# csyxwei/FFWM

Measured on AMD Instinct MI355X. Metric: train img/s (128x128, full FFWM GAN step), higher is better.
Workload: dtype f32; 1 GPU; BASELINE configs[2]: full FFWM train step (netG+netD+flowNetF+flowNetB, all losses, 3x Adam), synthetic MultiPIE-shaped 128x128; batch_per_gpu=8, global_batch=8, parallelism=dp1, grad_buckets=10, bucket_MiB=64

## Files before the change

### ffwm_amd/csrc/conv_bwd.hip

```cpp
#include "common.hpp"

namespace ffwm {
namespace {

typedef float f32x16 __attribute__((ext_vector_type(16)));

struct WgGeo {
    int C, H, W;
    int K, Ho, Wo;
    int stride, pad;
    int N;
    int P;
    int chunks_per_img;
    int chunks;
    int total_chunks;
    unsigned a_bytes, x_bytes;
};

constexpr int kPC = 32;
constexpr int kWAP = kPC + 1;
constexpr int kWBP = 65;

template <int R, int S>
__global__ void __launch_bounds__(kBlock)
conv_wgrad_generic_kernel(const float* __restrict__ a, const float* __restrict__ x, float* __restrict__ dw, const WgGeo g) {
    constexpr int RS = R * S;
    __shared__ float As[64 * kWAP];
    __shared__ float Bs[kPC * kWBP];
    const int lane = threadIdx.x & 63, wave = threadIdx.x >> 6;
    const int l31 = lane & 31, half = lane >> 5;
    const int wm = wave >> 1, wn = wave & 1;
    const int n0 = blockIdx.x * 64, k0 = blockIdx.y * 64;
    constexpr unsigned kOobOff = 0xFFFFFFF0u;
    const rsrc_t ra_ = make_rsrc(a, g.a_bytes);
    const rsrc_t rx_ = make_rsrc(x, g.x_bytes);
    const int HW = g.H * g.W;

    const int kk = threadIdx.x & 31, j0 = threadIdx.x >> 5;
    unsigned arow[8];
    int bc[8], br[8], bs[8];
#pragma unroll
    for (int i = 0; i < 8; ++i) {
        const int j = j0 + 8 * i;
        arow[i] = (k0 + j < g.K) ? static_cast<unsigned>(k0 + j) * static_cast<unsigned>(g.P) : kOobOff;
        const int n = n0 + j;
        if (n < g.N) {
            const int c = n / RS, rs = n - c * RS;
            bc[i] = c; br[i] = rs / S - g.pad; bs[i] = rs % S - g.pad;
        } else {
            bc[i] = -1; br[i] = 0; bs[i] = 0;
        }
    }

    const int ch_begin = blockIdx.z * g.chunks;
    const int ch_end = min(g.total_chunks, ch_begin + g.chunks);

    auto fetch = [&](int ch, float (&va)[8], float (&vb)[8]) {
        const int b = ch / g.chunks_per_img;
        const int p = (ch - b * g.chunks_per_img) * kPC + kk;
        const bool pin = p < g.P;
        const int oy = p / g.Wo, ox = p - oy * g.Wo;
        const int iy0 = oy * g.stride, ix0 = ox * g.stride;
        const unsigned abase = static_cast<unsigned>(b) * static_cast<unsigned>(g.K) * static_cast<unsigned>(g.P) + p;
        const unsigned xbase = static_cast<unsigned>(b) * static_cast<unsigned>(g.C) * static_cast<unsigned>(HW);
#pragma unroll
        for (int i = 0; i < 8; ++i) va[i] = buf_ld<float>(ra_, (pin && arow[i] != kOobOff) ? (abase + arow[i]) * 4u : kOobOff);
#pragma unroll
        for (int i = 0; i < 8; ++i) {
            const int iy = iy0 + br[i], ix = ix0 + bs[i];
            const bool ok = pin && bc[i] >= 0 && iy >= 0 && iy < g.H && ix >= 0 && ix < g.W;
            vb[i] = buf_ld<float>(rx_, ok ? (xbase + static_cast<unsigned>(bc[i]) * static_cast<unsigned>(HW) + static_cast<unsigned>(iy * g.W + ix)) * 4u
                                          : kOobOff);
        }
    };
    auto commit = [&](const float (&va)[8], const float (&vb)[8]) {
#pragma unroll
        for (int i = 0; i < 8; ++i) As[(j0 + 8 * i) * kWAP + kk] = va[i];
#pragma unroll
        for (int i = 0; i < 8; ++i) Bs[kk * kWBP + j0 + 8 * i] = vb[i];
    };

    f32x16 acc;
#pragma unroll
    for (int r = 0; r < 16; ++r) acc[r] = 0.f;
    auto compute = [&]() {
        const float* ap = As + (wm * 32 + l31) * kWAP + half;
        const float* bp = Bs + half * kWBP + wn * 32 + l31;
#pragma unroll
        for (int q = 0; q < kPC / 2; ++q)
            acc = __builtin_amdgcn_mfma_f32_32x32x2f32(ap[2 * q], bp[2 * q * kWBP], acc, 0, 0, 0);
    };

    float a0[8], b0[8], a1[8], b1[8];
    if (ch_begin < ch_end) fetch(ch_begin, a0, b0);
    if (ch_begin + 1 < ch_end) fetch(ch_begin + 1, a1, b1);
    for (int ch = ch_begin; ch < ch_end; ch += 2) {
        __syncthreads();
        commit(a0, b0);
        __syncthreads();
        if (ch + 2 < ch_end) fetch(ch + 2, a0, b0);
        compute();
        if (ch + 1 >= ch_end) break;
        __syncthreads();
        commit(a1, b1);
        __syncthreads();
        if (ch + 3 < ch_end) fetch(ch + 3, a1, b1);
        compute();
    }

    const int n = n0 + wn * 32 + l31;
    if (n >= g.N) return;
#pragma unroll
    for (int r = 0; r < 16; ++r) {
        const int k = k0 + wm * 32 + (r & 3) + 8 * (r >> 2) + 4 * half;
        if (k < g.K) atomic_add(dw + static_cast<size_t>(k) * g.N + n, acc[r]);
    }
}


struct Wg2Geo {
    int C, H, W, K, Ho, Wo, stride, pad;
    int N, P, HW;
    int total_px;
    int chunks_total;
    int chunks;
    int nz;
    unsigned a_bytes, x_bytes;
    FastDiv divP, divWo;
};

constexpr int kW2PC = 32;
constexpr int kW2P = 36;

template <int R, int S, int WM, int WN>
__global__ void __launch_bounds__(kBlock, 2)
conv_wgrad_tile_kernel(const float* __restrict__ a, const float* __restrict__ x, float* __restrict__ dw, float* __restrict__ gbias,
                       const Wg2Geo g) {
    constexpr int RS = R * S;
    constexpr int TM = 64 * WM, TN = 64 * WN;
    constexpr int NQA = TM * 8 / kBlock;
    constexpr int NXB = TN / 8;
    typedef float f32x4 __attribute__((ext_vector_type(4)));
    extern __shared__ __attribute__((aligned(16))) unsigned char smem_raw[];
    float* lds = reinterpret_cast<float*>(smem_raw);
    const int lane = threadIdx.x & 63, wave = threadIdx.x >> 6;
    const int l31 = lane & 31, half = lane >> 5;
    const int wm = wave >> 1, wn = wave & 1;
    const int n0 = blockIdx.x * TN, k0 = blockIdx.y * TM;
    constexpr unsigned kOobOff = 0xFFFFFFF0u;
    const rsrc_t ra_ = make_rsrc(a, g.a_bytes);
    const rsrc_t rx_ = make_rsrc(x, g.x_bytes);

    const int q8 = threadIdx.x & 7, arow0 = threadIdx.x >> 3;
    unsigned arow_off[NQA];
#pragma unroll
    for (int i = 0; i < NQA; ++i) {
        const int k = k0 + arow0 + 32 * i;
        arow_off[i] = k < g.K ? static_cast<unsigned>(k) * static_cast<unsigned>(g.P) : kOobOff;
    }
    const int kk = threadIdx.x & 31, xcol0 = threadIdx.x >> 5;
    int coloff[NXB];
    unsigned colsh[NXB];
#pragma unroll
    for (int i = 0; i < NXB; ++i) {
        const int n = n0 + xcol0 + 8 * i;
        const bool cin = n < g.N;
        const int nc = cin ? n : 0;
        const int c = nc / RS, rs = nc - c * RS;
        const int r = rs / S, sx = rs - r * S;
        coloff[i] = c * g.HW + r * g.W + sx;
        colsh[i] = cin ? static_cast<unsigned>(8 * r + sx) : 31u;
    }

    const int ch_begin = blockIdx.z * g.chunks;
    const int ch_end = min(g.chunks_total, ch_begin + g.chunks);
    const bool want_bias = gbias != nullptr && blockIdx.x == 0;

    f32x4 va[NQA];
    float vx[NXB];
    float bsum[NQA];
#pragma unroll
    for (int i = 0; i < NQA; ++i) bsum[i] = 0.f;

    unsigned a_base, a_pin;
    int x_base;
    int x_inv;
    auto prep = [&](int ch) {
        {
            const unsigned gq = static_cast<unsigned>(ch) * kW2PC + q8 * 4;
            const unsigned b = fast_div(gq, g.divP);
            const unsigned p = gq - b * static_cast<unsigned>(g.P);
            a_pin = 0u - static_cast<unsigned>(gq < static_cast<unsigned>(g.total_px));
            a_base = b * static_cast<unsigned>(g.K) * static_cast<unsigned>(g.P) + p;
        }
        {
            const unsigned gq = static_cast<unsigned>(ch) * kW2PC + kk;
            const unsigned b = fast_div(gq, g.divP);
            const unsigned p = gq - b * static_cast<unsigned>(g.P);
            const unsigned pin = static_cast<unsigned>(gq < static_cast<unsigned>(g.total_px));
            const int oy = static_cast<int>(fast_div(p, g.divWo)), ox = static_cast<int>(p) - oy * g.Wo;
            const int iy0 = oy * g.stride - g.pad, ix0 = ox * g.stride - g.pad;
            unsigned rmask = 0, smask = 0;
#pragma unroll
            for (int r = 0; r < R; ++r) rmask |= static_cast<unsigned>(static_cast<unsigned>(iy0 + r) < static_cast<unsigned>(g.H)) << r;
#pragma unroll
            for (int q = 0; q < S; ++q) smask |= static_cast<unsigned>(static_cast<unsigned>(ix0 + q) < static_cast<unsigned>(g.W)) << q;
            unsigned taps = 0;
#pragma unroll
            for (int r = 0; r < R; ++r) taps |= (smask & (0u - ((rmask >> r) & 1u))) << (8 * r);
            x_inv = static_cast<int>(~(taps & (0u - pin)));
            x_base = static_cast<int>(b) * g.C * g.HW + iy0 * g.W + ix0;
        }
    };
    auto issue_a = [&](int i) {
        const unsigned live = a_pin & (0u - static_cast<unsigned>(arow_off[i] != kOobOff));
        const unsigned off = (((a_base + arow_off[i]) * 4u) & live) | (kOobOff & ~live);
        const u32x4 v = __builtin_amdgcn_raw_buffer_load_b128(ra_, off, 0, 0);
        va[i][0] = __uint_as_float(v.x); va[i][1] = __uint_as_float(v.y); va[i][2] = __uint_as_float(v.z); va[i][3] = __uint_as_float(v.w);
    };
    auto issue_x = [&](int i) {
        const unsigned dead = static_cast<unsigned>(__builtin_amdgcn_sbfe(x_inv, colsh[i], 1u));
        vx[i] = buf_ld<float>(rx_, (static_cast<unsigned>(x_base + coloff[i]) << 2) | dead);
    };
    auto fetch = [&](int ch) {
        prep(ch);
#pragma unroll
        for (int i = 0; i < NQA; ++i) issue_a(i);
#pragma unroll
        for (int i = 0; i < NXB; ++i) issue_x(i);
    };
    auto commit = [&](int buf) {
        float* As = lds + buf * (TM + TN) * kW2P;
        float* Xs = As + TM * kW2P;
#pragma unroll
        for (int i = 0; i < NQA; ++i) {
            *reinterpret_cast<f32x4*>(As + (arow0 + 32 * i) * kW2P + q8 * 4) = va[i];
            if (want_bias) bsum[i] += (va[i][0] + va[i][1]) + (va[i][2] + va[i][3]);
        }
#pragma unroll
        for (int i = 0; i < NXB; ++i) Xs[(xcol0 + 8 * i) * kW2P + kk] = vx[i];
    };

    f32x16 acc[WM][WN];
#pragma unroll
    for (int i = 0; i < WM; ++i)
#pragma unroll
        for (int j = 0; j < WN; ++j)
#pragma unroll
            for (int r = 0; r < 16; ++r) acc[i][j][r] = 0.f;

    auto compute = [&](int buf, int next) {
        const float* As = lds + buf * (TM + TN) * kW2P;
        const float* Xs = As + TM * kW2P;
        const float* ap = As + (wm * 32 * WM + l31) * kW2P + 4 * half;
        const float* bp = Xs + (wn * 32 * WN + l31) * kW2P + 4 * half;
        if (next >= 0) prep(next);
#pragma unroll
        for (int gq = 0; gq < kW2PC / 8; ++gq) {
            f32x4 av[WM], bv[WN];
#pragma unroll
            for (int i = 0; i < WM; ++i) av[i] = *reinterpret_cast<const f32x4*>(ap + i * 32 * kW2P + 8 * gq);
#pragma unroll
            for (int j = 0; j < WN; ++j) bv[j] = *reinterpret_cast<const f32x4*>(bp + j * 32 * kW2P + 8 * gq);
            if (next >= 0) {
#pragma unroll
                for (int i = 0; i < NQA; ++i)
                    if (i % 4 == gq) issue_a(i);
#pragma unroll
                for (int i = 0; i < NXB; ++i)
                    if (i / (NXB / 4) == gq) issue_x(i);
            }
#pragma unroll
            for (int q = 0; q < 4; ++q)
#pragma unroll
                for (int i = 0; i < WM; ++i)
#pragma unroll
                    for (int j = 0; j < WN; ++j)
                        acc[i][j] = __builtin_amdgcn_mfma_f32_32x32x2f32(av[i][q], bv[j][q], acc[i][j], 0, 0, 0);
            __builtin_amdgcn_sched_barrier(0);
        }
    };

    if (ch_begin < ch_end) {
        fetch(ch_begin);
        commit(0);
        if (ch_begin + 1 < ch_end) fetch(ch_begin + 1);
        __syncthreads();
        for (int ch = ch_begin; ch < ch_end; ++ch) {
            const int cur = (ch - ch_begin) & 1;
            if (ch + 1 < ch_end) commit(cur ^ 1);
            compute(cur, ch + 2 < ch_end ? ch + 2 : -1);
            __syncthreads();
        }
    }

#pragma unroll
    for (int j = 0; j < WN; ++j) {
        const int n = n0 + wn * 32 * WN + j * 32 + l31;
        if (n >= g.N) continue;
#pragma unroll
        for (int i = 0; i < WM; ++i)
#pragma unroll
            for (int r = 0; r < 16; ++r) {
                const int k = k0 + wm * 32 * WM + i * 32 + (r & 3) + 8 * (r >> 2) + 4 * half;
                if (k >= g.K) continue;
                float* d = dw + static_cast<size_t>(k) * g.N + n;
                if (g.nz > 1) atomic_add(d, acc[i][j][r]);
                else *d = acc[i][j][r];
            }
    }
    if (want_bias) {
#pragma unroll
        for (int i = 0; i < NQA; ++i) {
            float v = bsum[i];
            v += __shfl_xor(v, 1, 64);
            v += __shfl_xor(v, 2, 64);
            v += __shfl_xor(v, 4, 64);
            const int k = k0 + arow0 + 32 * i;
            if (q8 == 0 && k < g.K) {
                if (g.nz > 1) atomic_add(gbias + k, v);
                else gbias[k] = v;
            }
        }
    }
}

}
}

using namespace ffwm;

extern "C" int ffwm_conv2d_wgrad(const void* rows, const void* gathered, void* grad_weight, int64_t B, int64_t K, int64_t Ho,
                                 int64_t Wo, int64_t C, int64_t H, int64_t W, int kernel, int stride, int pad, int dtype, void* stream) {
    const char* fn = "ffwm_conv2d_wgrad";
    FFWM_REQUIRE(dtype == FFWM_F32, FFWM_ERR_DTYPE, "%s: float32 only", fn);
    FFWM_REQUIRE(rows && gathered && grad_weight, FFWM_ERR_ARG, "%s: NULL tensor pointer", fn);
    FFWM_REQUIRE(B > 0 && K > 0 && C > 0 && Ho > 0 && Wo > 0 && H > 0 && W > 0, FFWM_ERR_ARG, "%s: sizes must be positive", fn);
    FFWM_REQUIRE((kernel == 1 || kernel == 3 || kernel == 4) && (stride == 1 || stride == 2) && pad >= 0 && pad < kernel, FFWM_ERR_ARG,
                 "%s: 1x1 / 3x3 / 4x4 kernels with stride 1 / 2 only", fn);
    FFWM_REQUIRE(Ho == (H + 2 * pad - kernel) / stride + 1 && Wo == (W + 2 * pad - kernel) / stride + 1, FFWM_ERR_ARG,
                 "%s: the row tensor's plane (%lld x %lld) is not the output plane of this convolution over %lld x %lld", fn,
                 (long long)Ho, (long long)Wo, (long long)H, (long long)W);
    FFWM_REQUIRE(B * K * Ho * Wo < (1LL << 29) && B * C * H * W < (1LL << 29), FFWM_ERR_SIZE, "%s: tensors must stay below 2 GiB", fn);
    WgGeo g;
    g.C = static_cast<int>(C); g.H = static_cast<int>(H); g.W = static_cast<int>(W);
    g.K = static_cast<int>(K); g.Ho = static_cast<int>(Ho); g.Wo = static_cast<int>(Wo);
    g.stride = stride; g.pad = pad;
    g.N = g.C * kernel * kernel;
    g.P = g.Ho * g.Wo;
    g.chunks_per_img = (g.P + kPC - 1) / kPC;
    g.total_chunks = static_cast<int>(B) * g.chunks_per_img;
    g.a_bytes = static_cast<unsigned>(B * K * Ho * Wo * 4);
    g.x_bytes = static_cast<unsigned>(B * C * H * W * 4);
    const int n_tiles = (g.N + 63) / 64, k_tiles = (g.K + 63) / 64;
    int64_t slices = (1024 + static_cast<int64_t>(n_tiles) * k_tiles - 1) / (static_cast<int64_t>(n_tiles) * k_tiles);
    if (slices > g.total_chunks / 4) slices = g.total_chunks / 4;
    if (slices < 1) slices = 1;
    g.chunks = static_cast<int>((g.total_chunks + slices - 1) / slices);
    const unsigned nz = static_cast<unsigned>((g.total_chunks + g.chunks - 1) / g.chunks);
    hipStream_t st = static_cast<hipStream_t>(stream);
    const double flops = 2.0 * B * g.P * static_cast<double>(g.K) * g.N;
    const double bytes = 4.0 * (static_cast<double>(B) * K * g.P + static_cast<double>(B) * C * H * W + static_cast<double>(K) * g.N);
    LaunchScope ls("conv_wgrad_mfma_generic", st, bytes, flops);
    const dim3 grid(static_cast<unsigned>(n_tiles), static_cast<unsigned>(k_tiles), nz);
    const float* a = static_cast<const float*>(rows);
    const float* x = static_cast<const float*>(gathered);
    float* dw = static_cast<float*>(grad_weight);
    if (kernel == 3) hipLaunchKernelGGL((conv_wgrad_generic_kernel<3, 3>), grid, dim3(kBlock), 0, st, a, x, dw, g);
    else if (kernel == 4) hipLaunchKernelGGL((conv_wgrad_generic_kernel<4, 4>), grid, dim3(kBlock), 0, st, a, x, dw, g);
    else hipLaunchKernelGGL((conv_wgrad_generic_kernel<1, 1>), grid, dim3(kBlock), 0, st, a, x, dw, g);
    return check_launch(fn);
}

extern "C" int ffwm_conv2d_wgrad_tiled(const void* rows, const void* gathered, void* grad_weight, void* grad_bias, int64_t B, int64_t K,
                                       int64_t Ho, int64_t Wo, int64_t C, int64_t H, int64_t W, int kernel, int stride, int pad,
                                       int prezeroed, int dtype, void* stream) {
    const char* fn = "ffwm_conv2d_wgrad_tiled";
    FFWM_REQUIRE(dtype == FFWM_F32, FFWM_ERR_DTYPE, "%s: float32 only", fn);
    FFWM_REQUIRE(rows && gathered && grad_weight, FFWM_ERR_ARG, "%s: NULL tensor pointer", fn);
    FFWM_REQUIRE(B > 0 && K > 0 && C > 0 && Ho > 0 && Wo > 0 && H > 0 && W > 0, FFWM_ERR_ARG, "%s: sizes must be positive", fn);
    FFWM_REQUIRE((kernel == 1 || kernel == 3 || kernel == 4) && (stride == 1 || stride == 2) && pad >= 0 && pad < kernel, FFWM_ERR_ARG,
                 "%s: 1x1 / 3x3 / 4x4 kernels with stride 1 / 2 only", fn);
    FFWM_REQUIRE(Ho == (H + 2 * pad - kernel) / stride + 1 && Wo == (W + 2 * pad - kernel) / stride + 1, FFWM_ERR_ARG,
                 "%s: the row tensor's plane (%lld x %lld) is not the output plane of this convolution over %lld x %lld", fn,
                 (long long)Ho, (long long)Wo, (long long)H, (long long)W);
    FFWM_REQUIRE((Ho * Wo) % 4 == 0, FFWM_ERR_ARG, "%s: the row tensor's plane must hold a multiple of 4 pixels", fn);
    FFWM_REQUIRE((reinterpret_cast<uintptr_t>(rows) & 15) == 0, FFWM_ERR_ARG, "%s: the row tensor must be 16-byte aligned", fn);
    FFWM_REQUIRE(B * K * Ho * Wo < (1LL << 29) && B * C * H * W < (1LL << 29), FFWM_ERR_SIZE, "%s: tensors must stay below 2 GiB", fn);
    Wg2Geo g;
    g.C = static_cast<int>(C); g.H = static_cast<int>(H); g.W = static_cast<int>(W);
    g.K = static_cast<int>(K); g.Ho = static_cast<int>(Ho); g.Wo = static_cast<int>(Wo);
    g.stride = stride; g.pad = pad;
    g.N = g.C * kernel * kernel;
    g.P = g.Ho * g.Wo;
    g.HW = g.H * g.W;
    g.total_px = static_cast<int>(B) * g.P;
    g.chunks_total = (g.total_px + kW2PC - 1) / kW2PC;
    g.a_bytes = static_cast<unsigned>(B * K * Ho * Wo * 4);
    g.x_bytes = static_cast<unsigned>(B * C * H * W * 4);
    g.divP = make_fast_div(static_cast<unsigned>(g.P));
    g.divWo = make_fast_div(static_cast<unsigned>(g.Wo));
    const int64_t wg_target = options().conv_wgrad_slice_target > 0 ? options().conv_wgrad_slice_target : 512;
    int wmt = 1, wnt = 1;
    double best = 1e30;
    for (int cm = 1; cm <= 2; ++cm)
        for (int cn = 1; cn <= 2; ++cn) {
            if ((cm == 2 && g.K <= 64) || (cn == 2 && g.N <= 64)) continue;
            const int64_t t = static_cast<int64_t>((g.K + 64 * cm - 1) / (64 * cm)) * ((g.N + 64 * cn - 1) / (64 * cn));
            int64_t sl = t >= wg_target ? 1 : wg_target / t;
            if (sl > g.chunks_total / 4) sl = g.chunks_total / 4;
            if (sl < 1) sl = 1;
            const int64_t per = (g.chunks_total + sl - 1) / sl;
            const int64_t nzc = (g.chunks_total + per - 1) / per;
            const int64_t rounds = (t * nzc + 511) / 512;
            const double est = rounds * (per * cm * cn * (cm * cn == 1 ? 1.6 : (cm * cn == 2 ? 1.25 : 1.0)) + 6.0 + (nzc > 1 ? 2.0 * cm * cn : 0.0));
            if (est < best) { best = est; wmt = cm; wnt = cn; }
        }
    const int k_tiles = (g.K + 64 * wmt - 1) / (64 * wmt), n_tiles = (g.N + 64 * wnt - 1) / (64 * wnt);
    const int64_t tiles = static_cast<int64_t>(k_tiles) * n_tiles;
    int64_t slices = tiles >= wg_target ? 1 : wg_target / tiles;
    if (slices > g.chunks_total / 4) slices = g.chunks_total / 4;
    if (slices < 1 || options().conv_wgrad_unsliced) slices = 1;
    g.chunks = static_cast<int>((g.chunks_total + slices - 1) / slices);
    g.nz = (g.chunks_total + g.chunks - 1) / g.chunks;
    hipStream_t st = static_cast<hipStream_t>(stream);
    float* dw = static_cast<float*>(grad_weight);
    float* gb = static_cast<float*>(grad_bias);
    if (g.nz > 1 && !prezeroed) {
        const size_t nw = static_cast<size_t>(g.K) * g.N;
        const bool joined = gb == dw + nw;
        if (zero_fill(dw, sizeof(float) * (nw + (joined ? static_cast<size_t>(g.K) : 0)), st)) return FFWM_ERR_LAUNCH;
        if (gb && !joined && zero_fill(gb, sizeof(float) * static_cast<size_t>(g.K), st)) return FFWM_ERR_LAUNCH;
    }
    const double flops = 2.0 * B * g.P * static_cast<double>(g.K) * g.N;
    const double bytes = 4.0 * (static_cast<double>(B) * K * g.P + static_cast<double>(B) * C * H * W + static_cast<double>(K) * g.N);
    LaunchScope ls("conv_wgrad_mfma_tiled", st, bytes, flops);
    const dim3 grid(static_cast<unsigned>(n_tiles), static_cast<unsigned>(k_tiles), static_cast<unsigned>(g.nz));
    const float* a = static_cast<const float*>(rows);
    const float* x = static_cast<const float*>(gathered);
#define FFWM_WG2(RR, MM, NN)                                                                                                  \
    do {                                                                                                                      \
        auto kfn = conv_wgrad_tile_kernel<RR, RR, MM, NN>;                                                                    \
        const size_t lds = 2u * (64 * MM + 64 * NN) * kW2P * sizeof(float);                                                   \
        allow_large_lds(reinterpret_cast<const void*>(kfn));                                                                  \
        hipLaunchKernelGGL(kfn, grid, dim3(kBlock), lds, st, a, x, dw, gb, g);                                                \
    } while (0)
#define FFWM_WG2_K(RR)                                                                                                        \
    do {                                                                                                                      \
        if (wmt == 2 && wnt == 2) FFWM_WG2(RR, 2, 2);                                                                         \
        else if (wmt == 2) FFWM_WG2(RR, 2, 1);                                                                                \
        else if (wnt == 2) FFWM_WG2(RR, 1, 2);                                                                                \
        else FFWM_WG2(RR, 1, 1);                                                                                              \
    } while (0)
    if (kernel == 3) FFWM_WG2_K(3);
    else if (kernel == 4) FFWM_WG2_K(4);
    else FFWM_WG2_K(1);
#undef FFWM_WG2_K
#undef FFWM_WG2
    return check_launch(fn);
}
```

Before: 214.3 img/s.

## Add row-staged 3x3 wgrad kernel that reuses input halo rows in LDS

Adds a new weight-gradient kernel for 3x3 pad-1 convolutions. It stages whole input row windows, with halo columns, per channel into LDS and derives all nine taps from that shared copy, so the input no longer has to be gathered once per (c,r,s) column. The N tiling changes from 64 im2col columns to 7 channels (63 columns), and the tile-size search and the dispatch are updated to match. In exchange it adds extra index math, LDS padding, a wasted column per tile and a larger code path, with possible register pressure given launch bounds of 2.

```diff
diff --git a/ffwm_amd/csrc/conv_bwd.hip b/ffwm_amd/csrc/conv_bwd.hip
--- a/ffwm_amd/csrc/conv_bwd.hip
+++ b/ffwm_amd/csrc/conv_bwd.hip
@@ -298,6 +298,270 @@
     for (int j = 0; j < WN; ++j) {
         const int n = n0 + wn * 32 * WN + j * 32 + l31;
         if (n >= g.N) continue;
+#pragma unroll
+        for (int i = 0; i < WM; ++i)
+#pragma unroll
+            for (int r = 0; r < 16; ++r) {
+                const int k = k0 + wm * 32 * WM + i * 32 + (r & 3) + 8 * (r >> 2) + 4 * half;
+                if (k >= g.K) continue;
+                float* d = dw + static_cast<size_t>(k) * g.N + n;
+                if (g.nz > 1) atomic_add(d, acc[i][j][r]);
+                else *d = acc[i][j][r];
+            }
+    }
+    if (want_bias) {
+#pragma unroll
+        for (int i = 0; i < NQA; ++i) {
+            float v = bsum[i];
+            v += __shfl_xor(v, 1, 64);
+            v += __shfl_xor(v, 2, 64);
+            v += __shfl_xor(v, 4, 64);
+            const int k = k0 + arow0 + 32 * i;
+            if (q8 == 0 && k < g.K) {
+                if (g.nz > 1) atomic_add(gbias + k, v);
+                else gbias[k] = v;
+            }
+        }
+    }
+}
+
+struct WgRowsGeo {
+    Wg2Geo g;
+    int cols, lcols;
+    int wr;
+    int qr;
+    int rp, cp;
+};
+
+constexpr int kWgRowsMaxLds = 80 * 1024;
+
+template <int STRIDE, int WN> struct WgRowsCfg {
+    static constexpr int NCH = 7 * WN;
+    static constexpr int NQX = STRIDE == 1 ? WN : WN + 1;
+    static constexpr int NHX = (STRIDE == 1 && WN == 2) ? 2 : 1;
+    static constexpr int NS = STRIDE == 1 ? 2 : 1;
+};
+
+template <int STRIDE, int WM, int WN>
+__global__ void __launch_bounds__(kBlock, 2)
+conv_wgrad_rows_kernel(const float* __restrict__ a, const float* __restrict__ x, float* __restrict__ dw, float* __restrict__ gbias,
+                       const WgRowsGeo gr) {
+    typedef WgRowsCfg<STRIDE, WN> Cfg;
+    constexpr int TM = 64 * WM;
+    constexpr int NCH = Cfg::NCH, NQX = Cfg::NQX, NHX = Cfg::NHX, NS = Cfg::NS;
+    constexpr int NQA = TM * 8 / kBlock;
+    typedef float f32x4 __attribute__((ext_vector_type(4)));
+    const Wg2Geo& g = gr.g;
+    extern __shared__ __attribute__((aligned(16))) unsigned char smem_raw[];
+    float* lds = reinterpret_cast<float*>(smem_raw);
+    float* const xs0 = lds + 2 * TM * kW2P;
+    const int xbuf = (NCH * gr.cp + 31) & ~31;
+    const int zoff = 2 * xbuf;
+    const int lane = threadIdx.x & 63, wave = threadIdx.x >> 6;
+    const int l31 = lane & 31, half = lane >> 5;
+    const int wm = wave >> 1, wn = wave & 1;
+    const int c0 = blockIdx.x * NCH, k0 = blockIdx.y * TM;
+    constexpr unsigned kOobOff = 0xFFFFFFF0u;
+    constexpr int kNoRow = 0x40000000;
+    const rsrc_t ra_ = make_rsrc(a, g.a_bytes);
+    const rsrc_t rx_ = make_rsrc(x, g.x_bytes);
+
+    const int q8 = threadIdx.x & 7, arow0 = threadIdx.x >> 3;
+    unsigned arow_off[NQA];
+#pragma unroll
+    for (int i = 0; i < NQA; ++i) {
+        const int k = k0 + arow0 + 32 * i;
+        arow_off[i] = k < g.K ? static_cast<unsigned>(k) * static_cast<unsigned>(g.P) : kOobOff;
+    }
+    int xq_g[NQX], xq_row[NQX], xq_l[NQX];
+    {
+        const int per_c = gr.wr * gr.qr, ntask = NCH * per_c;
+#pragma unroll
+        for (int i = 0; i < NQX; ++i) {
+            const int t = threadIdx.x + kBlock * i;
+            const bool in = t < ntask;
+            const int tt = in ? t : 0;
+            const int c = tt / per_c, rem = tt - c * per_c;
+            const int row = rem / gr.qr, q = rem - row * gr.qr;
+            xq_g[i] = c * g.HW + row * g.W + 4 * q;
+            xq_row[i] = (in && c0 + c < g.C) ? row : kNoRow;
+            xq_l[i] = in ? c * gr.cp + row * gr.rp + 1 + 4 * q : zoff;
+        }
+    }
+    int xh_g[NHX], xh_row[NHX], xh_l[NHX];
+    unsigned xh_right = 0;
+    {
+        const int per_c = gr.wr * NS, ntask = NCH * per_c;
+        const int xr = gr.cols * STRIDE;
+#pragma unroll
+        for (int i = 0; i < NHX; ++i) {
+            const int t = threadIdx.x + kBlock * i;
+            const bool in = t < ntask;
+            const int tt = in ? t : 0;
+            const int c = tt / per_c, rem = tt - c * per_c;
+            const int row = rem / NS, side = rem - row * NS;
+            xh_g[i] = c * g.HW + row * g.W + (side ? xr : -1);
+            xh_row[i] = (in && c0 + c < g.C) ? row : kNoRow;
+            xh_l[i] = in ? c * gr.cp + row * gr.rp + (side ? xr + 1 : 0) : zoff;
+            xh_right |= static_cast<unsigned>(side) << i;
+        }
+    }
+    int lb[2][WN];
+#pragma unroll
+    for (int j = 0; j < WN; ++j) {
+        const int n = wn * 32 * WN + j * 32 + l31;
+        const int c = n / 9, rs = n - 9 * c;
+        const int r = rs / 3, s = rs - 3 * r;
+        const int o = r * gr.rp + s;
+        lb[0][j] = c < NCH ? c * gr.cp + o : zoff + ((9 * NCH) & 31) + o;
+        lb[1][j] = c < NCH ? xbuf + c * gr.cp + o : zoff + ((9 * NCH) & 31) + o;
+    }
+    int poff[kW2PC / 8];
+#pragma unroll
+    for (int gq = 0; gq < kW2PC / 8; ++gq) {
+        const int px = 8 * gq + 4 * half;
+        poff[gq] = (px >> gr.lcols) * STRIDE * gr.rp + (px & (gr.cols - 1)) * STRIDE;
+    }
+
+    const int ch_begin = blockIdx.z * g.chunks;
+    const int ch_end = min(g.chunks_total, ch_begin + g.chunks);
+    const bool want_bias = gbias != nullptr && blockIdx.x == 0;
+
+    f32x4 va[NQA];
+    u32x4 vq[NQX];
+    float vh[NHX];
+    float bsum[NQA];
+#pragma unroll
+    for (int i = 0; i < NQA; ++i) bsum[i] = 0.f;
+
+    unsigned a_base, a_pin;
+    int x_base, x_iy0;
+    unsigned x_ldead, x_rdead;
+    auto prep = [&](int ch) {
+        {
+            const unsigned gq = static_cast<unsigned>(ch) * kW2PC + q8 * 4;
+            const unsigned b = fast_div(gq, g.divP);
+            const unsigned p = gq - b * static_cast<unsigned>(g.P);
+            a_pin = 0u - static_cast<unsigned>(gq < static_cast<unsigned>(g.total_px));
+            a_base = b * static_cast<unsigned>(g.K) * static_cast<unsigned>(g.P) + p;
+        }
+        {
+            const unsigned gq = static_cast<unsigned>(ch) * kW2PC;
+            const unsigned b = fast_div(gq, g.divP);
+            const unsigned p = gq - b * static_cast<unsigned>(g.P);
+            const int oy = static_cast<int>(fast_div(p, g.divWo)), ox = static_cast<int>(p) - oy * g.Wo;
+            x_iy0 = oy * STRIDE - 1;
+            x_base = (static_cast<int>(b) * g.C + c0) * g.HW + x_iy0 * g.W + ox * STRIDE;
+            x_ldead = 0u - static_cast<unsigned>(ox == 0);
+            x_rdead = 0u - static_cast<unsigned>((ox + gr.cols) * STRIDE >= g.W);
+        }
+    };
+    auto issue_a = [&](int i) {
+        const unsigned live = a_pin & (0u - static_cast<unsigned>(arow_off[i] != kOobOff));
+        const unsigned off = (((a_base + arow_off[i]) * 4u) & live) | (kOobOff & ~live);
+        const u32x4 v = __builtin_amdgcn_raw_buffer_load_b128(ra_, off, 0, 0);
+        va[i][0] = __uint_as_float(v.x); va[i][1] = __uint_as_float(v.y); va[i][2] = __uint_as_float(v.z); va[i][3] = __uint_as_float(v.w);
+    };
+    auto issue_q = [&](int i) {
+        const unsigned dead = static_cast<unsigned>(x_iy0 + xq_row[i]) < static_cast<unsigned>(g.H) ? 0u : kOobOff;
+        vq[i] = __builtin_amdgcn_raw_buffer_load_b128(rx_, (static_cast<unsigned>(x_base + xq_g[i]) << 2) | dead, 0, 0);
+    };
+    auto issue_h = [&](int i) {
+        const unsigned side = ((xh_right >> i) & 1u) ? x_rdead : x_ldead;
+        const unsigned dead = static_cast<unsigned>(x_iy0 + xh_row[i]) < static_cast<unsigned>(g.H) ? side : ~0u;
+        vh[i] = buf_ld<float>(rx_, (static_cast<unsigned>(x_base + xh_g[i]) << 2) | dead);
+    };
+    auto fetch = [&](int ch) {
+        prep(ch);
+#pragma unroll
+        for (int i = 0; i < NQA; ++i) issue_a(i);
+#pragma unroll
+        for (int i = 0; i < NQX; ++i) issue_q(i);
+#pragma unroll
+        for (int i = 0; i < NHX; ++i) issue_h(i);
+    };
+    auto commit = [&](int buf) {
+        float* As = lds + buf * TM * kW2P;
+        float* Xs = xs0 + buf * xbuf;
+#pragma unroll
+        for (int i = 0; i < NQA; ++i) {
+            *reinterpret_cast<f32x4*>(As + (arow0 + 32 * i) * kW2P + q8 * 4) = va[i];
+            if (want_bias) bsum[i] += (va[i][0] + va[i][1]) + (va[i][2] + va[i][3]);
+        }
+#pragma unroll
+        for (int i = 0; i < NQX; ++i) {
+            float* d = (xq_l[i] == zoff ? xs0 : Xs) + xq_l[i];
+            d[0] = __uint_as_float(vq[i].x); d[1] = __uint_as_float(vq[i].y); d[2] = __uint_as_float(vq[i].z); d[3] = __uint_as_float(vq[i].w);
+        }
+#pragma unroll
+        for (int i = 0; i < NHX; ++i) (xh_l[i] == zoff ? xs0 : Xs)[xh_l[i]] = vh[i];
+    };
+
+    f32x16 acc[WM][WN];
+#pragma unroll
+    for (int i = 0; i < WM; ++i)
+#pragma unroll
+        for (int j = 0; j < WN; ++j)
+#pragma unroll
+            for (int r = 0; r < 16; ++r) acc[i][j][r] = 0.f;
+
+    auto compute = [&](int buf, int next) {
+        const float* ap = lds + buf * TM * kW2P + (wm * 32 * WM + l31) * kW2P + 4 * half;
+        if (next >= 0) prep(next);
+#pragma unroll
+        for (int gq = 0; gq < kW2PC / 8; ++gq) {
+            f32x4 av[WM];
+            float bv[WN][4];
+#pragma unroll
+            for (int i = 0; i < WM; ++i) av[i] = *reinterpret_cast<const f32x4*>(ap + i * 32 * kW2P + 8 * gq);
+#pragma unroll
+            for (int j = 0; j < WN; ++j) {
+                const float* bp = xs0 + (buf ? lb[1][j] : lb[0][j]) + poff[gq];
+#pragma unroll
+                for (int q = 0; q < 4; ++q) bv[j][q] = bp[q * STRIDE];
+            }
+            if (next >= 0) {
+#pragma unroll
+                for (int i = 0; i < NQA; ++i)
+                    if (i % 4 == gq) issue_a(i);
+#pragma unroll
+                for (int i = 0; i < NQX; ++i)
+                    if (i == gq) issue_q(i);
+#pragma unroll
+                for (int i = 0; i < NHX; ++i)
+                    if (3 - i == gq) issue_h(i);
+            }
+#pragma unroll
+            for (int q = 0; q < 4; ++q)
+#pragma unroll
+                for (int i = 0; i < WM; ++i)
+#pragma unroll
+                    for (int j = 0; j < WN; ++j)
+                        acc[i][j] = __builtin_amdgcn_mfma_f32_32x32x2f32(av[i][q], bv[j][q], acc[i][j], 0, 0, 0);
+            __builtin_amdgcn_sched_barrier(0);
+        }
+    };
+
+    for (int i = threadIdx.x; i < gr.cp + 32; i += kBlock) xs0[zoff + i] = 0.f;
+    if (ch_begin < ch_end) {
+        fetch(ch_begin);
+        commit(0);
+        if (ch_begin + 1 < ch_end) fetch(ch_begin + 1);
+        __syncthreads();
+        for (int ch = ch_begin; ch < ch_end; ++ch) {
+            const int cur = (ch - ch_begin) & 1;
+            if (ch + 1 < ch_end) commit(cur ^ 1);
+            compute(cur, ch + 2 < ch_end ? ch + 2 : -1);
+            __syncthreads();
+        }
+    }
+
+#pragma unroll
+    for (int j = 0; j < WN; ++j) {
+        const int nl = wn * 32 * WN + j * 32 + l31;
+        const int c = nl / 9;
+        if (c >= NCH || c0 + c >= g.C) continue;
+        const int n = c0 * 9 + nl;
 #pragma unroll
         for (int i = 0; i < WM; ++i)
 #pragma unroll
@@ -400,13 +664,36 @@
     g.x_bytes = static_cast<unsigned>(B * C * H * W * 4);
     g.divP = make_fast_div(static_cast<unsigned>(g.P));
     g.divWo = make_fast_div(static_cast<unsigned>(g.Wo));
+    WgRowsGeo gr;
+    bool staged = false;
+    if (kernel == 3 && pad == 1 && W == Wo * stride && (reinterpret_cast<uintptr_t>(gathered) & 15) == 0) {
+        const int cols = Wo % 32 == 0 ? 32 : ((Wo >= 4 && 32 % Wo == 0 && Ho % (32 / Wo) == 0) ? static_cast<int>(Wo) : 0);
+        if (cols) {
+            gr.cols = cols;
+            gr.lcols = cols == 32 ? 5 : (cols == 16 ? 4 : (cols == 8 ? 3 : 2));
+            gr.wr = (32 / cols - 1) * stride + 3;
+            gr.qr = cols * stride / 4;
+            gr.rp = cols * stride + 2 <= 35 ? 35 : 67;
+            gr.cp = gr.wr * gr.rp;
+            gr.cp += (9 - gr.cp % 32 + 32) % 32;
+            staged = true;
+        }
+    }
+    auto rows_lds = [&](int cm, int cn) { return sizeof(float) * (2u * 64 * cm * kW2P + 2u * ((7u * cn * gr.cp + 31u) & ~31u) + gr.cp + 32u); };
+    auto rows_fits = [&](int cm, int cn) {
+        const int nqx = stride == 1 ? cn : cn + 1, nhx = (stride == 1 && cn == 2) ? 2 : 1, ns = stride == 1 ? 2 : 1;
+        return rows_lds(cm, cn) <= static_cast<size_t>(kWgRowsMaxLds) && 7 * cn * gr.wr * gr.qr <= kBlock * nqx && 7 * cn * gr.wr * ns <= kBlock * nhx;
+    };
+    if (staged && !rows_fits(1, 1)) staged = false;
     const int64_t wg_target = options().conv_wgrad_slice_target > 0 ? options().conv_wgrad_slice_target : 512;
     int wmt = 1, wnt = 1;
     double best = 1e30;
     for (int cm = 1; cm <= 2; ++cm)
         for (int cn = 1; cn <= 2; ++cn) {
-            if ((cm == 2 && g.K <= 64) || (cn == 2 && g.N <= 64)) continue;
-            const int64_t t = static_cast<int64_t>((g.K + 64 * cm - 1) / (64 * cm)) * ((g.N + 64 * cn - 1) / (64 * cn));
+            if (cm == 2 && g.K <= 64) continue;
+            if (staged ? (cn == 2 && g.C <= 7) || !rows_fits(cm, cn) : (cn == 2 && g.N <= 64)) continue;
+            const int64_t nt = staged ? (g.C + 7 * cn - 1) / (7 * cn) : (g.N + 64 * cn - 1) / (64 * cn);
+            const int64_t t = static_cast<int64_t>((g.K + 64 * cm - 1) / (64 * cm)) * nt;
             int64_t sl = t >= wg_target ? 1 : wg_target / t;
             if (sl > g.chunks_total / 4) sl = g.chunks_total / 4;
             if (sl < 1) sl = 1;
@@ -416,7 +703,8 @@
             const double est = rounds * (per * cm * cn * (cm * cn == 1 ? 1.6 : (cm * cn == 2 ? 1.25 : 1.0)) + 6.0 + (nzc > 1 ? 2.0 * cm * cn : 0.0));
             if (est < best) { best = est; wmt = cm; wnt = cn; }
         }
-    const int k_tiles = (g.K + 64 * wmt - 1) / (64 * wmt), n_tiles = (g.N + 64 * wnt - 1) / (64 * wnt);
+    const int k_tiles = (g.K + 64 * wmt - 1) / (64 * wmt);
+    const int n_tiles = staged ? (g.C + 7 * wnt - 1) / (7 * wnt) : (g.N + 64 * wnt - 1) / (64 * wnt);
     const int64_t tiles = static_cast<int64_t>(k_tiles) * n_tiles;
     int64_t slices = tiles >= wg_target ? 1 : wg_target / tiles;
     if (slices > g.chunks_total / 4) slices = g.chunks_total / 4;
@@ -452,9 +740,28 @@
         else if (wnt == 2) FFWM_WG2(RR, 1, 2);                                                                                \
         else FFWM_WG2(RR, 1, 1);                                                                                              \
     } while (0)
-    if (kernel == 3) FFWM_WG2_K(3);
+#define FFWM_WGR(SS, MM, NN)                                                                                                  \
+    do {                                                                                                                      \
+        auto kfn = conv_wgrad_rows_kernel<SS, MM, NN>;                                                                        \
+        allow_large_lds(reinterpret_cast<const void*>(kfn));                                                                  \
+        hipLaunchKernelGGL(kfn, grid, dim3(kBlock), rows_lds(MM, NN), st, a, x, dw, gb, gr);                                  \
+    } while (0)
+#define FFWM_WGR_S(SS)                                                                                                        \
+    do {                                                                                                                      \
+        if (wmt == 2 && wnt == 2) FFWM_WGR(SS, 2, 2);                                                                         \
+        else if (wmt == 2) FFWM_WGR(SS, 2, 1);                                                                                \
+        else if (wnt == 2) FFWM_WGR(SS, 1, 2);                                                                                \
+        else FFWM_WGR(SS, 1, 1);                                                                                              \
+    } while (0)
+    if (staged) {
+        gr.g = g;
+        if (stride == 1) FFWM_WGR_S(1);
+        else FFWM_WGR_S(2);
+    } else if (kernel == 3) FFWM_WG2_K(3);
     else if (kernel == 4) FFWM_WG2_K(4);
     else FFWM_WG2_K(1);
+#undef FFWM_WGR_S
+#undef FFWM_WGR
 #undef FFWM_WG2_K
 #undef FFWM_WG2
     return check_launch(fn);
```

After: 213.6 img/s. Within noise of the previous version (-0.3%).
